# AbnerVictor/OOD-GAN-inversion

Hardware: AMD Instinct MI355X
Metric: 1024² face inversions/sec (100 W+ steps) (higher is better)
Workload: dtype f16-split (hi+lo f16 operands, f32 accumulate): 3 MFMA/product in every forward conv (fp32-equivalent), 2 in the input-gradient convs (back-propagated gradient rounded to f16 before each contraction, weights keep hi+lo); dL/dW+ vs the float64 reference 1.4e-5..3.6e-5 ('f16s': 1.3e-5..2.6e-5, the ref

## Files before the change

ood-gan-inversion_amd/csrc/common.hpp:

```cpp
#pragma once
#include <hip/hip_runtime.h>
#include <cstdio>
#include <cstdarg>
#include <functional>
#include <utility>
#include "../../include/oodgan.h"

namespace oodgan {
struct PlanRec;
extern thread_local PlanRec* tl_plan_rec;
extern int g_null_launch;
void plan_append(std::function<void()>&& f);
template <class F>
inline void launch_rec(F&& f) {
    f();
    if (__builtin_expect(tl_plan_rec != nullptr, 0)) plan_append(std::function<void()>(std::forward<F>(f)));
}
}
#undef hipLaunchKernelGGL
#define hipLaunchKernelGGL(kernelName, numBlocks, numThreads, memPerBlock, streamId, ...)                                        \
    ::oodgan::launch_rec([=]() {                                                                                                 \
        if (!::oodgan::g_null_launch) (kernelName)<<<(numBlocks), (numThreads), (memPerBlock), (streamId)>>>(__VA_ARGS__);      \
    })

namespace oodgan {

void set_error(const char* fmt, ...);

enum { OODGAN_TUN_S1_BIG_MIN_ITEMS = 0, OODGAN_TUN_S2_BIG_MIN_ITEMS, OODGAN_TUN_T2_BIG_MIN_ITEMS, OODGAN_TUN_BLURT_STRIP, OODGAN_TUN_BLUR_STRIP, OODGAN_TUN_UPVB_WAVES, OODGAN_TUN_FEWOUT_QUAD, OODGAN_TUN_TINY_MID_MAX, OODGAN_TUN_STRIPX_WAVES, OODGAN_TUN_COUNT };
long tunable(int id);

enum { OODGAN_DC_STRIPX = 0, OODGAN_DC_STRIP, OODGAN_DC_S1BIG, OODGAN_DC_S1V2, OODGAN_DC_S1PP, OODGAN_DC_TINY, OODGAN_DC_T2BIG,
       OODGAN_DC_T2V2, OODGAN_DC_T2GEN, OODGAN_DC_S2BIG, OODGAN_DC_S2V2, OODGAN_DC_S2GEN, OODGAN_DC_UPVB,
       OODGAN_DC_S1BIG_YS, OODGAN_DC_S2BIG_FUSE, OODGAN_DC_S2BIG_DOTXS,
       OODGAN_DC_S1BIG_G2, OODGAN_DC_S2BIG_G2, OODGAN_DC_STRIPX_G2, OODGAN_DC_S2BIG_XH, OODGAN_DC_S1BIG_XH,
       OODGAN_DC_COMPOSITE_MSE,
       OODGAN_DC_SSIM,
       OODGAN_DC_ROBUST,
       OODGAN_DC_AREA_POOL,
       OODGAN_DC_POOLED_PIXEL, OODGAN_DC_COUNT };
void count_dispatch(int id);

bool bound_device_ok(const char* what);

inline int check_launch(const char* what) {
    hipError_t e = hipGetLastError();
    if (e != hipSuccess) {
        set_error("%s: %s", what, hipGetErrorString(e));
        return OODGAN_E_LAUNCH;
    }
    return OODGAN_OK;
}

#define OODGAN_REQUIRE(cond, ...)          \
    do {                                    \
        if (!(cond)) {                      \
            oodgan::set_error(__VA_ARGS__); \
            return OODGAN_E_ARG;            \
        }                                   \
    } while (0)

constexpr float kSqrt2 = 1.4142135623730951f;
constexpr float kInvPos = 1.f / kSqrt2, kInvNeg = 1.f / (0.2f * kSqrt2);
constexpr int kWave = 64;

inline hipStream_t as_stream(void* s) { return reinterpret_cast<hipStream_t>(s); }

inline int stream_grid(long work_items, int block) {
    long g = (work_items + block - 1) / block;
    if (g > 2048) g = 2048;
    if (g < 1) g = 1;
    return static_cast<int>(g);
}

__device__ __forceinline__ float wave_sum(float v) {
#pragma unroll
    for (int o = 32; o > 0; o >>= 1) v += __shfl_xor(v, o, 64);
    return v;
}

__device__ __forceinline__ float row_sum16(const float* __restrict__ p, int n, int l) {
    float v[4];
// ... 119 lines not shown
```

ood-gan-inversion_amd/csrc/conv_f16s_s2big.hip:

```cpp
#include "conv_common.hpp"
#include "sform.hpp"
#include <cstdint>
#include <cstdlib>
#include <type_traits>

using namespace oodgan;

typedef _Float16 half8 __attribute__((ext_vector_type(8)));
typedef __attribute__((address_space(3))) void lds_void;

#ifdef OODGAN_CLOCK_STAMP
__device__ unsigned long long* g_s2big_stamp = nullptr;
__device__ long g_s2big_stamp_n = 0;
#define S2_STAMP(i) do { if (FUSE && (wave == 0 || wave == 7)) stv[i] = __builtin_amdgcn_s_memtime(); } while (0)
#else
#define S2_STAMP(i)
#endif

namespace {

constexpr int SB_ROWS = 9, SB_C = 33;
constexpr int SB_ROWSLOTS = 2 * SB_C * 4;
constexpr int SB_XSLOTS = SB_ROWS * SB_ROWSLOTS;
constexpr int SB_XPIECES = 40;
constexpr int SB_XBYTES = SB_XPIECES * 1024;

struct SPDims2 { int KC, Hq, Wq; long plane; };

__host__ __device__ inline SPDims2 sp_dims2(int C, int H, int W) {
    SPDims2 d;
    d.KC = (C + 15) / 16;
    d.Hq = (H + 7) / 8 * 8 + 2;
    d.Wq = (W + 31) / 32 * 32 + 2;
    d.plane = (long)d.Hq * d.Wq * 4;
    return d;
}

struct S2Big {
    oodgan_conv_args a;
    const uint4* xs;
    SPDims2 sp;
    const float* w_unscale;
    int Hout, Wout, tiles_x, tiles_y, mblocks, Mp;
    long out_plane;
    int ablate;
    oodgan_actbwd_fuse f;
    SDims yd;
};

template <int MH>
struct S2Cfg {
    static constexpr int RW = MH == 2 ? 2 : 1;
    static constexpr int NRG = 8 / RW;
    static constexpr int MBW = 64 * MH;
    static constexpr int TAPB = 4 * MBW * 16;
    static constexpr int PPT = TAPB / 1024;
    static constexpr int WA = 6 * PPT / 8, WB = (3 * PPT + 7) / 8;
    static constexpr int NA = 5 + WA, NB = 5 + WB;
    static constexpr int OFF_XA = 0, OFF_WA = SB_XBYTES, OFF_XB = OFF_WA + 6 * TAPB, OFF_WB = OFF_XB + SB_XBYTES;
    static constexpr int SMEM = OFF_WB + 3 * TAPB;
    static constexpr int OFF_CST = SMEM;
    static constexpr int SMEM_FUSE = SMEM + 8 * MBW * 4;
};

constexpr int vmcnt_imm(int n) { return ((n >> 4) & 3) << 14 | 0x0F70 | (n & 15); }

typedef _Float16 half2v __attribute__((ext_vector_type(2)));

template <bool DOT, int MH, bool FUSE = false, bool G2 = false>
__global__ __launch_bounds__(512) void conv_f16s_s2big_kernel(const S2Big p, const uint4* __restrict__ wpk16) {
    using C = S2Cfg<MH>;
    constexpr int RW = C::RW;
    extern __shared__ __attribute__((aligned(16))) unsigned char smem[];
    const oodgan_conv_args& a = p.a;
    const int tid = threadIdx.x, lane = tid & 63;
    const int wave = __builtin_amdgcn_readfirstlane(tid >> 6);
    const int l31 = lane & 31, half = lane >> 5;
    const int rg = wave % C::NRG, mh = wave / C::NRG;

#ifdef OODGAN_CLOCK_STAMP
    unsigned long long stv[8] = {0, 0, 0, 0, 0, 0, 0, 0};
#endif
    S2_STAMP(0);
    int w = xcd_remap(blockIdx.x, gridDim.x);
    const int mblk = w % p.mblocks;
    w /= p.mblocks;
    const int ntile = p.tiles_x * p.tiles_y;
    const int tile = w % ntile, b = w / ntile;
    const int ty = tile / p.tiles_x, tx = tile % p.tiles_x;
    const int r0 = ty * 8, c0 = tx * 32, m0 = mblk * C::MBW;
    const int H = p.Hout, W = p.Wout, M = a.M;

    const bool xh = G2 && a.x_hi_only == 2;
    unsigned offx[5];
    bool xok[5];
#pragma unroll
    for (int i = 0; i < 5; ++i) {
        int P = (wave + 8 * i) * 64 + lane;
        if (P >= SB_XSLOTS) P = SB_XSLOTS - 1;
        const int row = P / SB_ROWSLOTS, rem = P % SB_ROWSLOTS;
        const int px = rem / (SB_C * 4), q = rem % (SB_C * 4);
        const int c = q >> 2, s = ((q & 3) - ((c >> 2) & 3)) & 3;
        if (xh) {
            offx[i] = (unsigned)(((long)px * p.sp.plane + ((long)(r0 + row) * p.sp.Wq + (c0 + c)) * 2 + (s & 1)) * 16);
            xok[i] = s < 2;
        } else {
            offx[i] = (unsigned)(((long)px * p.sp.plane + ((long)(r0 + row) * p.sp.Wq + (c0 + c)) * 4 + s) * 16);
            xok[i] = true;
        }
    }
    const long plane_bytes = p.sp.plane * 16;
    const int grp = a.groups > 1 ? m0 / (M / a.groups) : 0;
    const unsigned char* xb = reinterpret_cast<const unsigned char*>(p.xs) + ((long)b * p.sp.KC + (long)grp * ((a.K + 15) / 16)) * 4 * plane_bytes;
    const unsigned char* wb = reinterpret_cast<const unsigned char*>(wpk16) + (long)m0 * 16;
    const unsigned lane16 = lane * 16;
    const long wchunk_bytes = (long)36 * p.Mp * 16;
    const long wrow_bytes = (long)p.Mp * 16;
    const int nchunk = (a.K + 15) / 16;
    const int nstage = 2 * nchunk;

    auto dma_piece = [&](int st, int j) {
        const int t = st >> 1, py = st & 1;
        if (j < 5) {
            unsigned char* dx_ = smem + (py ? C::OFF_XB : C::OFF_XA);
            const unsigned char* xsrc = xb + ((long)t * 4 + py * 2) * plane_bytes;
            if (!G2 || xok[j])
                __builtin_amdgcn_global_load_lds((const __attribute__((address_space(1))) void*)(xsrc + offx[j]),
                                                 (lds_void*)(dx_ + (wave + 8 * j) * 1024), 16, 0, 0);
            return;
        }
        const int i = j - 5;
        const int nw = py ? C::WB : C::WA, npieces = (py ? 3 : 6) * C::PPT;
        if (i >= nw) return;
        unsigned char* dw_ = smem + (py ? C::OFF_WB : C::OFF_WA);
        const unsigned char* wsrc = wb + (long)t * wchunk_bytes;
        int pw = wave + 8 * i;
        if (pw >= npieces) pw -= 8;
        const int sl = pw / C::PPT, q = pw % C::PPT;
        const int tap = py ? 3 + sl : (sl / 3) * 6 + sl % 3;
        const int row = (q * 64) / C::MBW, j0 = (q * 64) % C::MBW;
        const unsigned char* sb = wsrc + (long)(tap * 4 + row) * wrow_bytes + j0 * 16;
        __builtin_amdgcn_global_load_lds((const __attribute__((address_space(1))) void*)(sb + lane16), (lds_void*)(dw_ + pw * 1024), 16, 0, 0);
    };
    auto dma_stage = [&](int st) {
#pragma unroll
        for (int j = 0; j < C::NA; ++j) dma_piece(st, j);
    };

    f32x16 acc[2][RW];
#pragma unroll
    for (int mt = 0; mt < 2; ++mt)
#pragma unroll
        for (int nt = 0; nt < RW; ++nt)
#pragma unroll
            for (int r = 0; r < 16; ++r) acc[mt][nt][r] = 0.f;

    unsigned lrd[2][2];
#pragma unroll
    for (int dxs = 0; dxs < 2; ++dxs)
#pragma unroll
        for (int lo = 0; lo < 2; ++lo) {
            const int c = dxs + l31;
            lrd[dxs][lo] = c * 64 + (((half + 2 * lo + ((c >> 2) & 3)) & 3) << 4);
        }
    const unsigned lwf = (half * C::MBW + mh * 64 + l31) * 16;

    struct Frag { half8 ah[2], al[2], bh[RW], bl[RW]; };
    auto load_tap = [&](Frag& f, const unsigned char* lx, const unsigned char* lw, auto sl_c) {
        constexpr int sl = decltype(sl_c)::value;
        constexpr int arow = sl / 3, kx = sl % 3;
#pragma unroll
        for (int mt = 0; mt < 2; ++mt) {
            f.ah[mt] = *reinterpret_cast<const half8*>(lw + sl * C::TAPB + (0 * 2) * C::MBW * 16 + mt * 32 * 16);
            f.al[mt] = *reinterpret_cast<const half8*>(lw + sl * C::TAPB + (1 * 2) * C::MBW * 16 + mt * 32 * 16);
        }
#pragma unroll
        for (int nt = 0; nt < RW; ++nt) {
            const unsigned char* xr = lx + ((rg * RW + nt + arow) * 2 + (kx & 1)) * (SB_C * 64);
            f.bh[nt] = *reinterpret_cast<const half8*>(xr + lrd[kx >> 1][0]);
            if (!G2) f.bl[nt] = *reinterpret_cast<const half8*>(xr + lrd[kx >> 1][1]);
        }
    };
    auto mfma_tap = [&](const Frag& f) {
#pragma unroll
        for (int mt = 0; mt < 2; ++mt)
#pragma unroll
            for (int nt = 0; nt < RW; ++nt) acc[mt][nt] = __builtin_amdgcn_mfma_f32_32x32x16_f16(f.ah[mt], f.bh[nt], acc[mt][nt], 0, 0, 0);
        if (!G2) {
#pragma unroll
        for (int mt = 0; mt < 2; ++mt)
#pragma unroll
            for (int nt = 0; nt < RW; ++nt) acc[mt][nt] = __builtin_amdgcn_mfma_f32_32x32x16_f16(f.ah[mt], f.bl[nt], acc[mt][nt], 0, 0, 0);
        }
#pragma unroll
        for (int mt = 0; mt < 2; ++mt)
#pragma unroll
            for (int nt = 0; nt < RW; ++nt) acc[mt][nt] = __builtin_amdgcn_mfma_f32_32x32x16_f16(f.al[mt], f.bh[nt], acc[mt][nt], 0, 0, 0);
    };
#define S2B_IC(n) std::integral_constant<int, n>{}
#define S2B_SB() __builtin_amdgcn_sched_barrier(0)

    constexpr bool EARLY = FUSE && MH == 1;
    float eq0 = 0.f, eq1 = 0.f, eq2 = 0.f, enz = 0.f, edv[EARLY ? 2 : 1][16];
    bool eok = false;
    if constexpr (EARLY) {
        static_assert(!EARLY || RW == 1, "one row per wave");
        const oodgan_actbwd_fuse& f = p.f;
        const int px = c0 + l31, py_ = r0 + rg;
        const long HW = (long)H * W, pix = (long)py_ * W + px;
        eok = py_ < H && px < W;
        if (eok) {
            if (f.g_rgb) {
                const float* gr = f.g_rgb + (long)b * 3 * HW + pix;
                eq0 = gr[0]; eq1 = gr[HW]; eq2 = gr[2 * HW];
            }
            if (f.noise) enz = (f.noise_w ? f.noise_w[0] : 1.f) * f.noise[(long)(f.noise_batch > 1 ? b : 0) * HW + pix];
        }
        if (a.dotx_sform) {
#pragma unroll
            for (int mt = 0; mt < 2; ++mt)
#pragma unroll
                for (int blk = 0; blk < 2; ++blk) {
                    const int kc = min((m0 + mh * 64 + mt * 32) / 16 + blk, p.yd.KC - 1);
                    const unsigned char* rec = reinterpret_cast<const unsigned char*>(a.dotx) +
                        sform_unit(p.yd, b, kc, min(py_, H - 1), min(px, W - 1), 0) * 16 + 8 * half;
#pragma unroll
                    for (int sl = 0; sl < 4; ++sl) {
                        const float2 t = *reinterpret_cast<const float2*>(rec + 16 * sl);
                        edv[EARLY ? mt : 0][8 * blk + 2 * sl] = t.x;
                        edv[EARLY ? mt : 0][8 * blk + 2 * sl + 1] = t.y;
                    }
                }
        } else {
#pragma unroll
            for (int mt = 0; mt < 2; ++mt) {
                const float* dr = a.dotx + ((long)b * M + m0 + mh * 64 + mt * 32) * HW + pix;
#pragma unroll
                for (int r = 0; r < 16; ++r) {
                    const int ch = (r & 3) + 8 * (r >> 2) + 4 * half;
                    edv[EARLY ? mt : 0][r] = (eok && m0 + mh * 64 + mt * 32 + ch < M) ? dr[(long)ch * HW] : 0.f;
                }
            }
        }
    }

    float cv[8] = {0.f, 0.f, 0.f, 0.f, 0.f, 0.f, 0.f, 1.f};
    if constexpr (FUSE) {
        const oodgan_actbwd_fuse& f = p.f;
        if (tid < C::MBW) {
            const int m = min(m0 + tid, M - 1);
            cv[0] = a.out_scale ? a.out_scale[(long)b * a.out_scale_stride + m] : 1.f;
            if (f.g_rgb) {
                cv[1] = f.w_rgb[0 * M + m];
                cv[2] = f.w_rgb[1 * M + m];
                cv[3] = f.w_rgb[2 * M + m];
                cv[4] = f.s_rgb[(long)b * f.s_rgb_stride + m];
            }
            if (f.bias) cv[5] = f.bias[m];
            cv[6] = f.dscale[(long)b * f.dscale_stride + m];
            if (a.dotx_sform) {
                const float sc = a.dotx_scale[(long)b * a.dotx_scale_stride + m];
                cv[7] = sc != 0.f ? 1.f / sc : 0.f;
            }
        }
    }
    dma_stage(0);
    if constexpr (FUSE) {
        if (tid < C::MBW) {
            const oodgan_actbwd_fuse& f = p.f;
            float* cst = reinterpret_cast<float*>(smem + C::OFF_CST);
            const bool mok = m0 + tid < M;
            cst[0 * C::MBW + tid] = mok ? cv[0] : 0.f;
            cst[1 * C::MBW + tid] = mok ? cv[1] * f.rgb_scale : 0.f;
            cst[2 * C::MBW + tid] = mok ? cv[2] * f.rgb_scale : 0.f;
            cst[3 * C::MBW + tid] = mok ? cv[3] * f.rgb_scale : 0.f;
            cst[4 * C::MBW + tid] = mok ? cv[4] : 0.f;
            cst[5 * C::MBW + tid] = mok ? cv[5] : 0.f;
            cst[6 * C::MBW + tid] = mok ? cv[6] * f.mul2[1] : 0.f;
            cst[7 * C::MBW + tid] = mok ? cv[7] : 0.f;
            __builtin_amdgcn_s_waitcnt(0xC07F);
        }
    }
    S2_STAMP(1);
    for (int st = 0; st < nstage; ++st) {
        const int py = st & 1;
        __builtin_amdgcn_s_waitcnt(vmcnt_imm(0));
        __builtin_amdgcn_s_barrier();
        const bool pf = st + 1 < nstage && !(p.ablate & 2);
        if (p.ablate & 1) { if (pf) dma_stage(st + 1); continue; }
        const unsigned char* lx = smem + (py ? C::OFF_XB : C::OFF_XA);
        const unsigned char* lw = smem + (py ? C::OFF_WB : C::OFF_WA) + lwf;
        Frag f0, f1;
        if (MH == 2 && pf) dma_stage(st + 1);
#define S2B_DMA(j) if (MH == 1 && pf) dma_piece(st + 1, (j));
        load_tap(f0, lx, lw, S2B_IC(0));
        S2B_SB();
        if (py == 0) {
            load_tap(f1, lx, lw, S2B_IC(1)); S2B_DMA(0) S2B_DMA(1) S2B_SB(); mfma_tap(f0); S2B_SB();
            load_tap(f0, lx, lw, S2B_IC(2)); S2B_DMA(2) S2B_DMA(3) S2B_SB(); mfma_tap(f1); S2B_SB();
            load_tap(f1, lx, lw, S2B_IC(3)); S2B_DMA(4) S2B_SB(); mfma_tap(f0); S2B_SB();
            load_tap(f0, lx, lw, S2B_IC(4)); S2B_DMA(5) S2B_SB(); mfma_tap(f1); S2B_SB();
            load_tap(f1, lx, lw, S2B_IC(5)); S2B_DMA(6) S2B_SB(); mfma_tap(f0); S2B_SB();
            S2B_DMA(7) S2B_SB();
            mfma_tap(f1);
        } else {
            load_tap(f1, lx, lw, S2B_IC(1)); S2B_DMA(0) S2B_DMA(1) S2B_DMA(2) S2B_DMA(3) S2B_SB(); mfma_tap(f0); S2B_SB();
            load_tap(f0, lx, lw, S2B_IC(2)); S2B_DMA(4) S2B_DMA(5) S2B_DMA(6) S2B_DMA(7) S2B_SB(); mfma_tap(f1); S2B_SB();
            S2B_DMA(8) S2B_DMA(9) S2B_DMA(10) S2B_SB();
            mfma_tap(f0);
        }
#undef S2B_DMA
    }
    __builtin_amdgcn_s_barrier();
    S2_STAMP(2);
#undef S2B_IC
#undef S2B_SB

    if constexpr (FUSE) {
        static_assert(DOT, "the fused epilogue includes the dot");
        const oodgan_actbwd_fuse& f = p.f;
        float* red = reinterpret_cast<float*>(smem);
        float* cst = reinterpret_cast<float*>(smem + C::OFF_CST);
        const float us = (p.w_unscale ? p.w_unscale[0] : 1.f) * (a.in_mul2 ? a.in_mul2[0] : 1.f);
        const float rscale = f.mul2[1];
        const int px = c0 + l31;
        const long HW = (long)H * W;
        const float nw = f.noise ? (f.noise_w ? f.noise_w[0] : 1.f) : 0.f;
        float q0[RW], q1[RW], q2[RW], nzv[RW];
        bool okr[RW];
#pragma unroll
        for (int nt = 0; nt < RW; ++nt) {
            const int py_ = r0 + rg * RW + nt;
            okr[nt] = py_ < H && px < W;
            q0[nt] = q1[nt] = q2[nt] = nzv[nt] = 0.f;
            if constexpr (EARLY) {
                okr[nt] = eok; q0[nt] = eq0; q1[nt] = eq1; q2[nt] = eq2; nzv[nt] = enz;
            } else if (okr[nt]) {
                const long pix = (long)py_ * W + px;
                if (f.g_rgb) {
                    const float* gr = f.g_rgb + (long)b * 3 * HW + pix;
                    q0[nt] = gr[0]; q1[nt] = gr[HW]; q2[nt] = gr[2 * HW];
                }
                if (f.noise) nzv[nt] = nw * f.noise[(long)(f.noise_batch > 1 ? b : 0) * HW + pix];
            }
        }
        float vmaxv = 0.f;
#pragma unroll
        for (int mt = 0; mt < 2; ++mt) {
            if (MH == 2) __builtin_amdgcn_sched_barrier(0);
            const int chb = mh * 64 + mt * 32;
            float dv[RW][16];
            if (a.dotx_sform) {
#pragma unroll
                for (int nt = 0; nt < RW; ++nt) {
                    float raw[16];
                    if constexpr (EARLY) {
#pragma unroll
                        for (int i = 0; i < 16; ++i) raw[i] = edv[EARLY ? mt : 0][i];
                    } else {
                        const int py_ = r0 + rg * RW + nt;
#pragma unroll
                        for (int blk = 0; blk < 2; ++blk) {
                            const int kc = min((m0 + chb) / 16 + blk, p.yd.KC - 1);
                            const unsigned char* rec = reinterpret_cast<const unsigned char*>(a.dotx) +
                                sform_unit(p.yd, b, kc, min(py_, H - 1), min(px, W - 1), 0) * 16 + 8 * half;
#pragma unroll
                            for (int sl = 0; sl < 4; ++sl) {
                                const float2 t = *reinterpret_cast<const float2*>(rec + 16 * sl);
                                raw[8 * blk + 2 * sl] = t.x;
                                raw[8 * blk + 2 * sl + 1] = t.y;
                            }
                        }
                    }
#pragma unroll
                    for (int r = 0; r < 16; ++r) {
// ... 278 lines not shown

namespace oodgan {

int launch_s2_big(const oodgan_conv_args& a_in, const void* wpk16, const float* unscale, hipStream_t st) {
    S2Big p;
    p.a = a_in;
    oodgan_conv_args& a = p.a;
    p.Hout = (a.Hin - 1) / 2;
    p.Wout = (a.Win - 1) / 2;
    if (a.out_pitch == 0) a.out_pitch = p.Wout;
    p.out_plane = (long)p.Hout * a.out_pitch;
    p.xs = reinterpret_cast<const uint4*>(a.x);
    p.sp = sp_dims2(a.K * (a.groups > 1 ? a.groups : 1), p.Hout, p.Wout);
    p.w_unscale = unscale;
    p.tiles_y = (p.Hout + 7) / 8;
    p.tiles_x = (p.Wout + 31) / 32;
    p.Mp = (a.M + 63) / 64 * 64;
    const long items128 = (long)p.tiles_x * p.tiles_y * a.B * (a.M / 128);
    const bool mh2 = (a.M % 128) == 0 && items128 >= 256;
    p.mblocks = mh2 ? a.M / 128 : (a.M + 63) / 64;
    if (a.dotx) {
        OODGAN_REQUIRE(a.dot_part != nullptr, "conv3x3: dotx without dot_part");
        OODGAN_REQUIRE(a.dot_nparts == p.tiles_x * p.tiles_y, "conv3x3 f16s S2: dot_nparts %d != %d", a.dot_nparts, p.tiles_x * p.tiles_y);
    }
    OODGAN_REQUIRE((long)a.M * p.out_plane * 4 < (1L << 32), "conv3x3 S2 big: plane too large");
    const bool fuse = a.fuse != nullptr;
    p.yd = sform_dims(a.M, p.Hout, p.Wout);
    if (fuse) {
        p.f = *a.fuse;
        OODGAN_REQUIRE(a.dotx && a.dot_part && p.f.ys && p.f.part_r && p.f.part_max && p.f.dscale && p.f.mul2 && (a.M % 32) == 0,
                       "conv3x3 S2 fused activation backward: needs dotx, ys, part_r, part_max, dscale, mul2 and M %% 32 == 0");
        OODGAN_REQUIRE(!p.f.g_rgb || (p.f.w_rgb && p.f.s_rgb && p.f.part_t), "conv3x3 S2 fused: rgb branch needs w_rgb, s_rgb and part_t");
        OODGAN_REQUIRE(p.f.noise == nullptr || p.f.noise_batch == 1 || p.f.noise_batch == a.B, "conv3x3 S2 fused: noise_batch");
        OODGAN_REQUIRE(p.f.nmax >= (long)a.B * p.tiles_x * p.tiles_y * p.mblocks * 8, "conv3x3 S2 fused: part_max too small");
    }
    OODGAN_REQUIRE(p.sp.plane * 32 < (1L << 32), "conv3x3 S2 big: input plane too large");
#ifdef OODGAN_DEBUG_ABLATE
    static const int abl = getenv("OODGAN_S2BIG_ABLATE") ? atoi(getenv("OODGAN_S2BIG_ABLATE")) : 0;
    p.ablate = abl;
#else
    p.ablate = 0;
#endif
    const long total = (long)p.tiles_x * p.tiles_y * a.B * p.mblocks;
    OODGAN_REQUIRE(total > 0 && total < (1L << 31), "conv3x3: grid too large");
    static bool once = ((void)hipFuncSetAttribute(reinterpret_cast<const void*>(&conv_f16s_s2big_kernel<true, 2>), hipFuncAttributeMaxDynamicSharedMemorySize, S2Cfg<2>::SMEM),
                        (void)hipFuncSetAttribute(reinterpret_cast<const void*>(&conv_f16s_s2big_kernel<false, 2>), hipFuncAttributeMaxDynamicSharedMemorySize, S2Cfg<2>::SMEM),
                        (void)hipFuncSetAttribute(reinterpret_cast<const void*>(&conv_f16s_s2big_kernel<true, 1>), hipFuncAttributeMaxDynamicSharedMemorySize, S2Cfg<1>::SMEM),
                        (void)hipFuncSetAttribute(reinterpret_cast<const void*>(&conv_f16s_s2big_kernel<false, 1>), hipFuncAttributeMaxDynamicSharedMemorySize, S2Cfg<1>::SMEM),
                        (void)hipFuncSetAttribute(reinterpret_cast<const void*>(&conv_f16s_s2big_kernel<true, 2, true>), hipFuncAttributeMaxDynamicSharedMemorySize, S2Cfg<2>::SMEM_FUSE),
                        (void)hipFuncSetAttribute(reinterpret_cast<const void*>(&conv_f16s_s2big_kernel<true, 1, true>), hipFuncAttributeMaxDynamicSharedMemorySize, S2Cfg<1>::SMEM_FUSE),
                        (void)hipFuncSetAttribute(reinterpret_cast<const void*>(&conv_f16s_s2big_kernel<true, 2, false, true>), hipFuncAttributeMaxDynamicSharedMemorySize, S2Cfg<2>::SMEM),
                        (void)hipFuncSetAttribute(reinterpret_cast<const void*>(&conv_f16s_s2big_kernel<true, 1, false, true>), hipFuncAttributeMaxDynamicSharedMemorySize, S2Cfg<1>::SMEM),
                        (void)hipFuncSetAttribute(reinterpret_cast<const void*>(&conv_f16s_s2big_kernel<true, 2, true, true>), hipFuncAttributeMaxDynamicSharedMemorySize, S2Cfg<2>::SMEM_FUSE),
                        (void)hipFuncSetAttribute(reinterpret_cast<const void*>(&conv_f16s_s2big_kernel<true, 1, true, true>), hipFuncAttributeMaxDynamicSharedMemorySize, S2Cfg<1>::SMEM_FUSE), true);
    (void)once;
    const uint4* w16 = reinterpret_cast<const uint4*>(wpk16);
    const bool g2 = a.x_hi_only != 0 && a.dotx != nullptr;
    OODGAN_REQUIRE(a.x_hi_only != 2 || (g2 && a.groups <= 1), "conv3x3 S2 big: hi-only input records (x_hi_only = 2) need dotx (the two-instruction instances) and no groups");
    if (g2) {
        count_dispatch(OODGAN_DC_S2BIG_G2);
        if (a.x_hi_only == 2) count_dispatch(OODGAN_DC_S2BIG_XH);
        if (fuse) {
            if (mh2) hipLaunchKernelGGL((conv_f16s_s2big_kernel<true, 2, true, true>), dim3((unsigned)total), dim3(512), S2Cfg<2>::SMEM_FUSE, st, p, w16);
            else hipLaunchKernelGGL((conv_f16s_s2big_kernel<true, 1, true, true>), dim3((unsigned)total), dim3(512), S2Cfg<1>::SMEM_FUSE, st, p, w16);
        } else if (mh2) hipLaunchKernelGGL((conv_f16s_s2big_kernel<true, 2, false, true>), dim3((unsigned)total), dim3(512), S2Cfg<2>::SMEM, st, p, w16);
        else hipLaunchKernelGGL((conv_f16s_s2big_kernel<true, 1, false, true>), dim3((unsigned)total), dim3(512), S2Cfg<1>::SMEM, st, p, w16);
    } else if (fuse) {
        if (mh2) hipLaunchKernelGGL((conv_f16s_s2big_kernel<true, 2, true>), dim3((unsigned)total), dim3(512), S2Cfg<2>::SMEM_FUSE, st, p, w16);
        else hipLaunchKernelGGL((conv_f16s_s2big_kernel<true, 1, true>), dim3((unsigned)total), dim3(512), S2Cfg<1>::SMEM_FUSE, st, p, w16);
    } else if (mh2) {
        if (a.dotx) hipLaunchKernelGGL((conv_f16s_s2big_kernel<true, 2>), dim3((unsigned)total), dim3(512), S2Cfg<2>::SMEM, st, p, w16);
        else hipLaunchKernelGGL((conv_f16s_s2big_kernel<false, 2>), dim3((unsigned)total), dim3(512), S2Cfg<2>::SMEM, st, p, w16);
    } else {
        if (a.dotx) hipLaunchKernelGGL((conv_f16s_s2big_kernel<true, 1>), dim3((unsigned)total), dim3(512), S2Cfg<1>::SMEM, st, p, w16);
        else hipLaunchKernelGGL((conv_f16s_s2big_kernel<false, 1>), dim3((unsigned)total), dim3(512), S2Cfg<1>::SMEM, st, p, w16);
    }
    return check_launch("conv3x3_f16s_s2big");
}

}
```

ood-gan-inversion_amd/csrc/runtime.hip:

```cpp
#include "common.hpp"
#include <atomic>
#include <cstdlib>
#include <cstring>
#include <new>

namespace oodgan {
static thread_local char g_err[512] = "";
void set_error(const char* fmt, ...) {
    va_list ap;
    va_start(ap, fmt);
    vsnprintf(g_err, sizeof(g_err), fmt, ap);
    va_end(ap);
}
}

namespace oodgan {
namespace {
struct Tunable { const char* name; const char* env; long def; std::atomic<long> val; std::atomic<int> init; };
Tunable g_tun[OODGAN_TUN_COUNT] = {
    {"s1_big_min_items", "OODGAN_S1_BIG_MIN_ITEMS", 128, {0}, {0}},
    {"s2_big_min_items", "OODGAN_S2_BIG_MIN_ITEMS", 128, {0}, {0}},
    {"t2_big_min_items", "OODGAN_T2_BIG_MIN_ITEMS", 128, {0}, {0}},
    {"blurt_strip", "OODGAN_BLURT_STRIP", 1, {0}, {0}},
    {"blur_strip", "OODGAN_BLUR_STRIP", 1, {0}, {0}},
    {"upvb_waves", "OODGAN_UPVB_WAVES", 12, {0}, {0}},
    {"fewout_quad", "OODGAN_FEWOUT_QUAD", 1, {0}, {0}},
    {"tiny_mid_max", "OODGAN_TINY_MID_MAX", 1024, {0}, {0}},
    {"stripx_waves", "OODGAN_STRIPX_WAVES", 4, {0}, {0}},
};
}
long tunable(int id) {
    Tunable& t = g_tun[id];
    if (!t.init.load(std::memory_order_acquire)) {
        const char* e = getenv(t.env);
        t.val.store(e ? atol(e) : t.def, std::memory_order_relaxed);
        t.init.store(1, std::memory_order_release);
    }
    return t.val.load(std::memory_order_relaxed);
}
}

extern "C" int oodgan_set_tunable(const char* name, long value) {
    OODGAN_REQUIRE(name != nullptr, "set_tunable: null name");
    for (int i = 0; i < oodgan::OODGAN_TUN_COUNT; ++i)
        if (strcmp(name, oodgan::g_tun[i].name) == 0) {
            oodgan::g_tun[i].val.store(value, std::memory_order_relaxed);
            oodgan::g_tun[i].init.store(1, std::memory_order_release);
            return OODGAN_OK;
        }
    oodgan::set_error("set_tunable: unknown tunable '%s'", name);
    return OODGAN_E_ARG;
}
extern "C" long oodgan_get_tunable(const char* name) {
    if (name)
        for (int i = 0; i < oodgan::OODGAN_TUN_COUNT; ++i)
            if (strcmp(name, oodgan::g_tun[i].name) == 0) return oodgan::tunable(i);
    return -1;
}

namespace oodgan {
bool bound_device_ok(const char* what) {
    static std::atomic<int> bound{-1};
    int dev = 0;
    if (hipGetDevice(&dev) != hipSuccess) {
        (void)hipGetLastError();
        set_error("%s: no current HIP device", what);
        return false;
    }
    int expected = -1;
    if (bound.compare_exchange_strong(expected, dev, std::memory_order_acq_rel) || expected == dev) return true;
    set_error("%s: liboodgan_hip.so is bound to HIP device %d (its first use in this process) but device %d is current — one process per GPU "
              "(select the device with HIP_VISIBLE_DEVICES or torch.cuda.set_device before the first call)", what, expected, dev);
    return false;
}
}

namespace oodgan {
namespace {
const char* const g_dc_name[OODGAN_DC_COUNT] = {"stripx", "strip", "s1big", "s1v2", "s1pp", "tiny", "t2big", "t2v2", "t2gen", "s2big", "s2v2", "s2gen", "upvb", "s1big_ys", "s2big_fuse", "s2big_dotx_sform", "s1big_g2", "s2big_g2", "stripx_g2", "s2big_xh", "s1big_xh", "composite_mse", "ssim", "robust", "area_pool", "pooled_pixel"};
std::atomic<long> g_dc[OODGAN_DC_COUNT];
}
// ... 98 lines not shown
```

ood-gan-inversion_amd/csrc/upfirdn2d.hip:

```cpp
#include "common.hpp"

using namespace oodgan;

namespace {

struct UfdArgs {
    const float* x;
    const float* k;
    float* y;
    const float* bias;
    const float* noise;
    const float* noise_w;
    int planes, C;
    int in_h, in_w, in_pitch;
    int out_h, out_w, out_pitch;
    int kh, kw, up_x, up_y, down_x, down_y, pad_x0, pad_y0;
    int noise_batch, act;
};

__global__ __launch_bounds__(256) void generic_kernel(const UfdArgs a) {
    const long total = (long)a.planes * a.out_h * a.out_w;
    const long in_plane = (long)a.in_h * a.in_pitch, out_plane = (long)a.out_h * a.out_pitch;
    for (long e = blockIdx.x * (long)blockDim.x + threadIdx.x; e < total; e += (long)gridDim.x * blockDim.x) {
        const int ox = (int)(e % a.out_w);
        const int oy = (int)((e / a.out_w) % a.out_h);
        const long pl = e / ((long)a.out_w * a.out_h);
        const float* xp = a.x + pl * in_plane;
        float acc = 0.f;
        for (int ky = 0; ky < a.kh; ++ky) {
            const int u = oy * a.down_y + ky - a.pad_y0;
            if (u < 0 || u % a.up_y) continue;
            const int iy = u / a.up_y;
            if (iy >= a.in_h) continue;
            for (int kx = 0; kx < a.kw; ++kx) {
                const int v = ox * a.down_x + kx - a.pad_x0;
                if (v < 0 || v % a.up_x) continue;
                const int ix = v / a.up_x;
                if (ix >= a.in_w) continue;
                acc += a.k[(a.kh - 1 - ky) * a.kw + (a.kw - 1 - kx)] * xp[(long)iy * a.in_pitch + ix];
            }
        }
        if (a.noise) {
            const long b = pl / a.C;
            acc += (a.noise_w ? a.noise_w[0] : 1.f) * a.noise[(a.noise_batch > 1 ? b : 0) * (long)a.out_h * a.out_w + (long)oy * a.out_w + ox];
        }
        if (a.bias) acc += a.bias[pl % a.C];
        if (a.act == OODGAN_ACT_LRELU) acc = (acc > 0.f ? acc : 0.2f * acc) * kSqrt2;
        a.y[pl * out_plane + (long)oy * a.out_pitch + ox] = acc;
    }
}

__global__ __launch_bounds__(256) void down2_k4_kernel(const UfdArgs a) {
    __shared__ float kf[16];
    if (threadIdx.x < 16) kf[threadIdx.x] = a.k[15 - threadIdx.x];
    __syncthreads();
    const long total = (long)a.planes * a.out_h * a.out_w;
    const long in_plane = (long)a.in_h * a.in_pitch, out_plane = (long)a.out_h * a.out_pitch;
    for (long e = blockIdx.x * 256L + threadIdx.x; e < total; e += (long)gridDim.x * 256) {
        const int ox = (int)(e % a.out_w);
        const int oy = (int)((e / a.out_w) % a.out_h);
        const long pl = e / ((long)a.out_w * a.out_h);
        const float* xp = a.x + pl * in_plane;
        const int y0 = 2 * oy - a.pad_y0, x0 = 2 * ox - a.pad_x0;
        float v[16];
#pragma unroll
        for (int ky = 0; ky < 4; ++ky)
#pragma unroll
            for (int kx = 0; kx < 4; ++kx)
                v[ky * 4 + kx] = xp[(long)min(max(y0 + ky, 0), a.in_h - 1) * a.in_pitch + min(max(x0 + kx, 0), a.in_w - 1)];
        float acc = 0.f;
#pragma unroll
        for (int ky = 0; ky < 4; ++ky)
#pragma unroll
            for (int kx = 0; kx < 4; ++kx) {
                const int iy = y0 + ky, ix = x0 + kx;
                if (iy >= 0 && iy < a.in_h && ix >= 0 && ix < a.in_w) acc += kf[ky * 4 + kx] * v[ky * 4 + kx];
            }
        a.y[pl * out_plane + (long)oy * a.out_pitch + ox] = acc;
    }
}

constexpr int FT_H = 32, FT_W = 64, FK = 4;
constexpr int FL_H = FT_H + FK - 1, FL_W = FT_W + FK - 1;
constexpr int FL_P = FL_W + 1;

__global__ __launch_bounds__(256) void fir_tile_kernel(const UfdArgs a, int tiles_x, int tiles_y) {
    __shared__ float t[FL_H * FL_P];
    __shared__ float kf[FK * FK];
    int w = blockIdx.x;
    const int tx_ = w % tiles_x; w /= tiles_x;
    const int ty_ = w % tiles_y; w /= tiles_y;
    const long pl = w;
    const int oy0 = ty_ * FT_H, ox0 = tx_ * FT_W;
    const long in_plane = (long)a.in_h * a.in_pitch, out_plane = (long)a.out_h * a.out_pitch;
    const float* xp = a.x + pl * in_plane;
    if (threadIdx.x < FK * FK) {
        const int ky = threadIdx.x / FK, kx = threadIdx.x % FK;
        kf[threadIdx.x] = (ky < a.kh && kx < a.kw) ? a.k[(a.kh - 1 - ky) * a.kw + (a.kw - 1 - kx)] : 0.f;
    }
    const int iy0 = oy0 - a.pad_y0, ix0 = ox0 - a.pad_x0;
    {
        constexpr int NF = (FL_H * FL_W + 255) / 256;
        float fv[NF];
#pragma unroll
        for (int i = 0; i < NF; ++i) {
            const int e = min((int)threadIdx.x + 256 * i, FL_H * FL_W - 1);
            const int iy = iy0 + e / FL_W, ix = ix0 + e % FL_W;
            fv[i] = xp[(long)min(max(iy, 0), a.in_h - 1) * a.in_pitch + min(max(ix, 0), a.in_w - 1)];
        }
#pragma unroll
        for (int i = 0; i < NF; ++i) {
            const int e = (int)threadIdx.x + 256 * i;
            if (e >= FL_H * FL_W) continue;
            const int r = e / FL_W, c = e % FL_W;
            const int iy = iy0 + r, ix = ix0 + c;
            t[r * FL_P + c] = (iy >= 0 && iy < a.in_h && ix >= 0 && ix < a.in_w) ? fv[i] : 0.f;
        }
    }
    __syncthreads();
    const int tx = threadIdx.x & 15, ty = threadIdx.x >> 4;
    float kr[FK * FK];
#pragma unroll
    for (int i = 0; i < FK * FK; ++i) kr[i] = kf[i];
    const long b = pl / a.C;
    const float bv = a.bias ? a.bias[pl % a.C] : 0.f;
    const float nw = a.noise ? (a.noise_w ? a.noise_w[0] : 1.f) : 0.f;
    const float* np = a.noise ? a.noise + (a.noise_batch > 1 ? b : 0) * (long)a.out_h * a.out_w : nullptr;
    float nzv[2][4];
#pragma unroll
    for (int rr = 0; rr < 2; ++rr)
#pragma unroll
        for (int j = 0; j < 4; ++j) {
            const int oy = min(oy0 + ty + rr * 16, a.out_h - 1), ox = min(ox0 + 4 * tx + j, a.out_w - 1);
            nzv[rr][j] = *(np ? np + (long)oy * a.out_w + ox : xp);
        }
#pragma unroll
    for (int rr = 0; rr < 2; ++rr) {
        const int r = ty + rr * 16;
        float o[4] = {0.f, 0.f, 0.f, 0.f};
#pragma unroll
        for (int ky = 0; ky < FK; ++ky) {
            float row[4 + FK - 1];
#pragma unroll
            for (int j = 0; j < 4 + FK - 1; ++j) row[j] = t[(r + ky) * FL_P + 4 * tx + j];
#pragma unroll
            for (int kx = 0; kx < FK; ++kx)
#pragma unroll
                for (int j = 0; j < 4; ++j) o[j] += kr[ky * FK + kx] * row[j + kx];
        }
        const int oy = oy0 + r;
        if (oy >= a.out_h) continue;
#pragma unroll
        for (int j = 0; j < 4; ++j) {
            const int ox = ox0 + 4 * tx + j;
            if (ox >= a.out_w) continue;
            float v = o[j];
            if (np) v += nw * nzv[rr][j];
            v += bv;
            if (a.act == OODGAN_ACT_LRELU) v = (v > 0.f ? v : 0.2f * v) * kSqrt2;
            a.y[pl * out_plane + (long)oy * a.out_pitch + ox] = v;
        }
    }
}

int run(UfdArgs& a, int pad_x1, int pad_y1, hipStream_t st) {
    OODGAN_REQUIRE(a.x && a.k && a.y, "upfirdn2d: null tensor");
    OODGAN_REQUIRE(a.planes > 0 && a.in_h > 0 && a.in_w > 0 && a.kh > 0 && a.kw > 0, "upfirdn2d: bad shape");
    OODGAN_REQUIRE(a.up_x >= 1 && a.up_y >= 1 && a.down_x >= 1 && a.down_y >= 1, "upfirdn2d: up/down must be >= 1");
    a.out_h = (a.in_h * a.up_y + a.pad_y0 + pad_y1 - a.kh) / a.down_y + 1;
    a.out_w = (a.in_w * a.up_x + a.pad_x0 + pad_x1 - a.kw) / a.down_x + 1;
    OODGAN_REQUIRE(a.out_h > 0 && a.out_w > 0, "upfirdn2d: empty output (%d x %d)", a.out_h, a.out_w);
    if (a.in_pitch == 0) a.in_pitch = a.in_w;
    if (a.out_pitch == 0) a.out_pitch = a.out_w;
    OODGAN_REQUIRE(a.in_pitch >= a.in_w && a.out_pitch >= a.out_w, "upfirdn2d: pitch smaller than width");
    const bool tiled = a.up_x == 1 && a.up_y == 1 && a.down_x == 1 && a.down_y == 1 && a.kh <= FK && a.kw <= FK &&
                       (long)a.out_h * a.out_w >= 64 * 64;
    if (tiled) {
        const int tiles_x = (a.out_w + FT_W - 1) / FT_W, tiles_y = (a.out_h + FT_H - 1) / FT_H;
        const long nb = (long)tiles_x * tiles_y * a.planes;
        OODGAN_REQUIRE(nb < (1L << 31), "upfirdn2d: grid too large");
        hipLaunchKernelGGL(fir_tile_kernel, dim3((unsigned)nb), dim3(256), 0, st, a, tiles_x, tiles_y);
    } else if (a.up_x == 1 && a.up_y == 1 && a.down_x == 2 && a.down_y == 2 && a.kh == 4 && a.kw == 4 && !a.noise && !a.bias &&
               a.act == OODGAN_ACT_NONE) {
        const long total = (long)a.planes * a.out_h * a.out_w;
        hipLaunchKernelGGL(down2_k4_kernel, dim3(stream_grid(total, 256)), dim3(256), 0, st, a);
    } else {
        const long total = (long)a.planes * a.out_h * a.out_w;
        hipLaunchKernelGGL(generic_kernel, dim3(stream_grid(total, 256)), dim3(256), 0, st, a);
    }
    return check_launch("upfirdn2d");
}

}

extern "C" int oodgan_upfirdn2d(const float* x, const float* kernel, float* y, int planes, int in_h, int in_w, int in_pitch,
                                int out_pitch, int kh, int kw, int up_x, int up_y, int down_x, int down_y, int pad_x0,
                                int pad_x1, int pad_y0, int pad_y1, void* stream) {
    UfdArgs a{};
    a.x = x; a.k = kernel; a.y = y;
    a.planes = planes; a.C = 1;
    a.in_h = in_h; a.in_w = in_w; a.in_pitch = in_pitch; a.out_pitch = out_pitch;
    a.kh = kh; a.kw = kw; a.up_x = up_x; a.up_y = up_y; a.down_x = down_x; a.down_y = down_y;
    a.pad_x0 = pad_x0; a.pad_y0 = pad_y0;
    a.act = OODGAN_ACT_NONE; a.noise_batch = 1;
    return run(a, pad_x1, pad_y1, as_stream(stream));
}

extern "C" int oodgan_blur_bias_act(const float* x, const float* kernel, float* y, int B, int C, int in_h, int in_w,
                                    int in_pitch, int kh, int kw, int pad0, int pad1, const float* bias, const float* noise,
                                    int noise_batch, const float* noise_w, int act, void* stream) {
    OODGAN_REQUIRE(B > 0 && C > 0, "blur_bias_act: bad batch/channels");
    OODGAN_REQUIRE(noise == nullptr || noise_batch == 1 || noise_batch == B, "blur_bias_act: noise_batch");
    UfdArgs a{};
    a.x = x; a.k = kernel; a.y = y;
    a.planes = B * C; a.C = C;
    a.in_h = in_h; a.in_w = in_w; a.in_pitch = in_pitch; a.out_pitch = 0;
    a.kh = kh; a.kw = kw; a.up_x = a.up_y = a.down_x = a.down_y = 1;
    a.pad_x0 = pad0; a.pad_y0 = pad0;
    a.bias = bias; a.noise = noise; a.noise_w = noise_w; a.noise_batch = noise_batch; a.act = act;
    return run(a, pad1, pad1, as_stream(stream));
}
```

Before: 7.897.

## Add resident-operand stride-2 conv path and vectorized down2 FIR kernel

Adds a resident-operand variant of the fused MH=1 stride-2 conv kernel. It DMAs every stage's input and weight tiles into LDS up front and then runs the MFMA stages behind staged vmcnt waits, replacing the per-stage load/wait loop. This is meant to overlap all global loads with compute for small-K layers, at the cost of a larger LDS footprint and so possibly lower occupancy. Separately, it adds a vectorized downsample-by-2 4x4 FIR kernel that computes four outputs per thread from float4 row loads, cutting redundant scalar loads. Both paths are gated by new tunables that default on.

Result: no change. 7.957 (median of 5 runs) (+0.8%).

```diff
diff --git a/ood-gan-inversion_amd/csrc/common.hpp b/ood-gan-inversion_amd/csrc/common.hpp
--- a/ood-gan-inversion_amd/csrc/common.hpp
+++ b/ood-gan-inversion_amd/csrc/common.hpp
@@ -27,7 +27,7 @@
 
 void set_error(const char* fmt, ...);
 
-enum { OODGAN_TUN_S1_BIG_MIN_ITEMS = 0, OODGAN_TUN_S2_BIG_MIN_ITEMS, OODGAN_TUN_T2_BIG_MIN_ITEMS, OODGAN_TUN_BLURT_STRIP, OODGAN_TUN_BLUR_STRIP, OODGAN_TUN_UPVB_WAVES, OODGAN_TUN_FEWOUT_QUAD, OODGAN_TUN_TINY_MID_MAX, OODGAN_TUN_STRIPX_WAVES, OODGAN_TUN_COUNT };
+enum { OODGAN_TUN_S1_BIG_MIN_ITEMS = 0, OODGAN_TUN_S2_BIG_MIN_ITEMS, OODGAN_TUN_T2_BIG_MIN_ITEMS, OODGAN_TUN_BLURT_STRIP, OODGAN_TUN_BLUR_STRIP, OODGAN_TUN_UPVB_WAVES, OODGAN_TUN_FEWOUT_QUAD, OODGAN_TUN_TINY_MID_MAX, OODGAN_TUN_STRIPX_WAVES, OODGAN_TUN_DOWN2_VEC, OODGAN_TUN_S2_RESIDENT, OODGAN_TUN_COUNT };
 long tunable(int id);
 
 enum { OODGAN_DC_STRIPX = 0, OODGAN_DC_STRIP, OODGAN_DC_S1BIG, OODGAN_DC_S1V2, OODGAN_DC_S1PP, OODGAN_DC_TINY, OODGAN_DC_T2BIG,
diff --git a/ood-gan-inversion_amd/csrc/conv_f16s_s2big.hip b/ood-gan-inversion_amd/csrc/conv_f16s_s2big.hip
--- a/ood-gan-inversion_amd/csrc/conv_f16s_s2big.hip
+++ b/ood-gan-inversion_amd/csrc/conv_f16s_s2big.hip
@@ -63,14 +63,25 @@
     static constexpr int SMEM_FUSE = SMEM + 8 * MBW * 4;
 };
 
+constexpr int RS_XSLOTS = SB_ROWS * 2 * SB_C * 2;
+constexpr int RS_XPIECES = 19;
+constexpr int RS_XREG = RS_XPIECES * 1024;
+constexpr int RS_TAPB = 4096;
+constexpr int RS_OFF_W = 4 * RS_XREG;
+constexpr int RS_OFF_CST = RS_OFF_W + 18 * RS_TAPB;
+constexpr int RS_SMEM = RS_OFF_CST + 8 * 64 * 4;
+constexpr int RS_NA = 6, RS_NB = 5;
+
 constexpr int vmcnt_imm(int n) { return ((n >> 4) & 3) << 14 | 0x0F70 | (n & 15); }
 
 typedef _Float16 half2v __attribute__((ext_vector_type(2)));
 
-template <bool DOT, int MH, bool FUSE = false, bool G2 = false>
+template <bool DOT, int MH, bool FUSE = false, bool G2 = false, bool RES = false>
 __global__ __launch_bounds__(512) void conv_f16s_s2big_kernel(const S2Big p, const uint4* __restrict__ wpk16) {
     using C = S2Cfg<MH>;
     constexpr int RW = C::RW;
+    static_assert(!RES || (MH == 1 && FUSE && G2), "the resident-operand form exists for the fused two-instruction MH = 1 instance");
+    constexpr int OFF_CST = RES ? RS_OFF_CST : C::OFF_CST;
     extern __shared__ __attribute__((aligned(16))) unsigned char smem[];
     const oodgan_conv_args& a = p.a;
     const int tid = threadIdx.x, lane = tid & 63;
@@ -94,6 +105,18 @@
     const bool xh = G2 && a.x_hi_only == 2;
     unsigned offx[5];
     bool xok[5];
+    if constexpr (RES) {
+#pragma unroll
+        for (int i = 0; i < 3; ++i) {
+            int P = min(wave + 8 * i, RS_XPIECES - 1) * 64 + lane;
+            if (P >= RS_XSLOTS) P = RS_XSLOTS - 1;
+            const int run = P / (2 * SB_C), q = P % (2 * SB_C);
+            const int row = run >> 1, px = run & 1, c = q >> 1, u = (q ^ (c >> 3)) & 1;
+            offx[i] = (unsigned)(((long)px * p.sp.plane + ((long)(r0 + row) * p.sp.Wq + (c0 + c)) * 2 + u) * 16);
+            xok[i] = true;
+        }
+        offx[3] = offx[4] = 0; xok[3] = xok[4] = false;
+    } else {
 #pragma unroll
     for (int i = 0; i < 5; ++i) {
         int P = (wave + 8 * i) * 64 + lane;
@@ -108,6 +131,7 @@
             offx[i] = (unsigned)(((long)px * p.sp.plane + ((long)(r0 + row) * p.sp.Wq + (c0 + c)) * 4 + s) * 16);
             xok[i] = true;
         }
+    }
     }
     const long plane_bytes = p.sp.plane * 16;
     const int grp = a.groups > 1 ? m0 / (M / a.groups) : 0;
@@ -181,6 +205,38 @@
             if (!G2) f.bl[nt] = *reinterpret_cast<const half8*>(xr + lrd[kx >> 1][1]);
         }
     };
+    const unsigned lrr0 = l31 * 32 + ((half ^ (l31 >> 3)) & 1) * 16, lrr1 = (l31 + 1) * 32 + ((half ^ ((l31 + 1) >> 3)) & 1) * 16;
+    auto load_tap_r = [&](Frag& f, const unsigned char* lx, const unsigned char* lw, auto py_c, auto sl_c) {
+        constexpr int sl = decltype(sl_c)::value, py = decltype(py_c)::value;
+        constexpr int arow = sl / 3, kx = sl % 3, tap = py ? 3 + sl : (sl / 3) * 6 + sl % 3;
+#pragma unroll
+        for (int mt = 0; mt < 2; ++mt) {
+            f.ah[mt] = *reinterpret_cast<const half8*>(lw + tap * RS_TAPB + (0 * 2) * 64 * 16 + mt * 32 * 16);
+            f.al[mt] = *reinterpret_cast<const half8*>(lw + tap * RS_TAPB + (1 * 2) * 64 * 16 + mt * 32 * 16);
+        }
+        f.bh[0] = *reinterpret_cast<const half8*>(lx + ((rg + arow) * 2 + (kx & 1)) * (SB_C * 32) + ((kx >> 1) ? lrr1 : lrr0));
+    };
+    auto dma_stage_r = [&](int st) {
+        const int t = st >> 1, py = st & 1;
+        const unsigned char* xsrc = xb + ((long)t * 4 + py * 2) * plane_bytes;
+#pragma unroll
+        for (int i = 0; i < 3; ++i)
+            __builtin_amdgcn_global_load_lds((const __attribute__((address_space(1))) void*)(xsrc + offx[i]),
+                                             (lds_void*)(smem + st * RS_XREG + min(wave + 8 * i, RS_XPIECES - 1) * 1024), 16, 0, 0);
+        const unsigned char* wsrc = wb + (long)t * wchunk_bytes;
+        const int nw = py ? 2 : 3;
+#pragma unroll
+        for (int i = 0; i < 3; ++i) {
+            if (i >= nw) break;
+            int pw = wave + 8 * i;
+            if (pw >= (py ? 12 : 24)) pw -= 8;
+            const int sl = pw >> 2, row = pw & 3;
+            const int tap = py ? 3 + sl : (sl / 3) * 6 + sl % 3;
+            const unsigned char* sb = wsrc + (long)(tap * 4 + row) * wrow_bytes;
+            __builtin_amdgcn_global_load_lds((const __attribute__((address_space(1))) void*)(sb + lane16),
+                                             (lds_void*)(smem + RS_OFF_W + (t * 9 + tap) * RS_TAPB + row * 1024), 16, 0, 0);
+        }
+    };
     auto mfma_tap = [&](const Frag& f) {
 #pragma unroll
         for (int mt = 0; mt < 2; ++mt)
@@ -264,11 +320,17 @@
             }
         }
     }
-    dma_stage(0);
-    if constexpr (FUSE) {
+    if constexpr (RES) {
+        S2B_SB();
+        for (int st = 0; st < nstage; ++st) dma_stage_r(st);
+        S2B_SB();
+    } else {
+        dma_stage(0);
+    }
+    auto park_cst = [&]() {
         if (tid < C::MBW) {
             const oodgan_actbwd_fuse& f = p.f;
-            float* cst = reinterpret_cast<float*>(smem + C::OFF_CST);
+            float* cst = reinterpret_cast<float*>(smem + OFF_CST);
             const bool mok = m0 + tid < M;
             cst[0 * C::MBW + tid] = mok ? cv[0] : 0.f;
             cst[1 * C::MBW + tid] = mok ? cv[1] * f.rgb_scale : 0.f;
@@ -280,8 +342,45 @@
             cst[7 * C::MBW + tid] = mok ? cv[7] : 0.f;
             __builtin_amdgcn_s_waitcnt(0xC07F);
         }
-    }
+    };
+    if constexpr (FUSE && !RES) park_cst();
     S2_STAMP(1);
+    if constexpr (RES) {
+        auto stage_a = [&](int t) {
+            const unsigned char* lx = smem + (2 * t) * RS_XREG;
+            const unsigned char* lw = smem + RS_OFF_W + t * 9 * RS_TAPB + lwf;
+            Frag f0, f1;
+            load_tap_r(f0, lx, lw, S2B_IC(0), S2B_IC(0));
+            S2B_SB();
+            load_tap_r(f1, lx, lw, S2B_IC(0), S2B_IC(1)); S2B_SB(); mfma_tap(f0); S2B_SB();
+            load_tap_r(f0, lx, lw, S2B_IC(0), S2B_IC(2)); S2B_SB(); mfma_tap(f1); S2B_SB();
+            load_tap_r(f1, lx, lw, S2B_IC(0), S2B_IC(3)); S2B_SB(); mfma_tap(f0); S2B_SB();
+            load_tap_r(f0, lx, lw, S2B_IC(0), S2B_IC(4)); S2B_SB(); mfma_tap(f1); S2B_SB();
+            load_tap_r(f1, lx, lw, S2B_IC(0), S2B_IC(5)); S2B_SB(); mfma_tap(f0); S2B_SB();
+            mfma_tap(f1);
+        };
+        auto stage_b = [&](int t) {
+            const unsigned char* lx = smem + (2 * t + 1) * RS_XREG;
+            const unsigned char* lw = smem + RS_OFF_W + t * 9 * RS_TAPB + lwf;
+            Frag f0, f1;
+            load_tap_r(f0, lx, lw, S2B_IC(1), S2B_IC(0));
+            S2B_SB();
+            load_tap_r(f1, lx, lw, S2B_IC(1), S2B_IC(1)); S2B_SB(); mfma_tap(f0); S2B_SB();
+            load_tap_r(f0, lx, lw, S2B_IC(1), S2B_IC(2)); S2B_SB(); mfma_tap(f1); S2B_SB();
+            mfma_tap(f0);
+        };
+#define S2B_WAIT(n) do { S2B_SB(); __builtin_amdgcn_s_waitcnt(vmcnt_imm(n)); __builtin_amdgcn_s_barrier(); S2B_SB(); } while (0)
+        if (nchunk == 2) {
+            S2B_WAIT(RS_NB + RS_NA + RS_NB); stage_a(0);
+            S2B_WAIT(RS_NA + RS_NB); stage_b(0);
+            S2B_WAIT(RS_NB); stage_a(1);
+            S2B_WAIT(0); stage_b(1);
+        } else {
+            S2B_WAIT(RS_NB); stage_a(0);
+            S2B_WAIT(0); stage_b(0);
+        }
+#undef S2B_WAIT
+    } else
     for (int st = 0; st < nstage; ++st) {
         const int py = st & 1;
         __builtin_amdgcn_s_waitcnt(vmcnt_imm(0));
@@ -311,6 +410,7 @@
         }
 #undef S2B_DMA
     }
+    if constexpr (RES) park_cst();
     __builtin_amdgcn_s_barrier();
     S2_STAMP(2);
 #undef S2B_IC
@@ -320,7 +420,7 @@
         static_assert(DOT, "the fused epilogue includes the dot");
         const oodgan_actbwd_fuse& f = p.f;
         float* red = reinterpret_cast<float*>(smem);
-        float* cst = reinterpret_cast<float*>(smem + C::OFF_CST);
+        float* cst = reinterpret_cast<float*>(smem + OFF_CST);
         const float us = (p.w_unscale ? p.w_unscale[0] : 1.f) * (a.in_mul2 ? a.in_mul2[0] : 1.f);
         const float rscale = f.mul2[1];
         const int px = c0 + l31;
@@ -705,7 +805,8 @@
                         (void)hipFuncSetAttribute(reinterpret_cast<const void*>(&conv_f16s_s2big_kernel<true, 2, false, true>), hipFuncAttributeMaxDynamicSharedMemorySize, S2Cfg<2>::SMEM),
                         (void)hipFuncSetAttribute(reinterpret_cast<const void*>(&conv_f16s_s2big_kernel<true, 1, false, true>), hipFuncAttributeMaxDynamicSharedMemorySize, S2Cfg<1>::SMEM),
                         (void)hipFuncSetAttribute(reinterpret_cast<const void*>(&conv_f16s_s2big_kernel<true, 2, true, true>), hipFuncAttributeMaxDynamicSharedMemorySize, S2Cfg<2>::SMEM_FUSE),
-                        (void)hipFuncSetAttribute(reinterpret_cast<const void*>(&conv_f16s_s2big_kernel<true, 1, true, true>), hipFuncAttributeMaxDynamicSharedMemorySize, S2Cfg<1>::SMEM_FUSE), true);
+                        (void)hipFuncSetAttribute(reinterpret_cast<const void*>(&conv_f16s_s2big_kernel<true, 1, true, true>), hipFuncAttributeMaxDynamicSharedMemorySize, S2Cfg<1>::SMEM_FUSE),
+                        (void)hipFuncSetAttribute(reinterpret_cast<const void*>(&conv_f16s_s2big_kernel<true, 1, true, true, true>), hipFuncAttributeMaxDynamicSharedMemorySize, RS_SMEM), true);
     (void)once;
     const uint4* w16 = reinterpret_cast<const uint4*>(wpk16);
     const bool g2 = a.x_hi_only != 0 && a.dotx != nullptr;
@@ -714,7 +815,9 @@
         count_dispatch(OODGAN_DC_S2BIG_G2);
         if (a.x_hi_only == 2) count_dispatch(OODGAN_DC_S2BIG_XH);
         if (fuse) {
+            const bool res = !mh2 && a.x_hi_only == 2 && a.K <= 32 && a.groups <= 1 && tunable(OODGAN_TUN_S2_RESIDENT) != 0;
             if (mh2) hipLaunchKernelGGL((conv_f16s_s2big_kernel<true, 2, true, true>), dim3((unsigned)total), dim3(512), S2Cfg<2>::SMEM_FUSE, st, p, w16);
+            else if (res) hipLaunchKernelGGL((conv_f16s_s2big_kernel<true, 1, true, true, true>), dim3((unsigned)total), dim3(512), RS_SMEM, st, p, w16);
             else hipLaunchKernelGGL((conv_f16s_s2big_kernel<true, 1, true, true>), dim3((unsigned)total), dim3(512), S2Cfg<1>::SMEM_FUSE, st, p, w16);
         } else if (mh2) hipLaunchKernelGGL((conv_f16s_s2big_kernel<true, 2, false, true>), dim3((unsigned)total), dim3(512), S2Cfg<2>::SMEM, st, p, w16);
         else hipLaunchKernelGGL((conv_f16s_s2big_kernel<true, 1, false, true>), dim3((unsigned)total), dim3(512), S2Cfg<1>::SMEM, st, p, w16);
diff --git a/ood-gan-inversion_amd/csrc/runtime.hip b/ood-gan-inversion_amd/csrc/runtime.hip
--- a/ood-gan-inversion_amd/csrc/runtime.hip
+++ b/ood-gan-inversion_amd/csrc/runtime.hip
@@ -27,6 +27,8 @@
     {"fewout_quad", "OODGAN_FEWOUT_QUAD", 1, {0}, {0}},
     {"tiny_mid_max", "OODGAN_TINY_MID_MAX", 1024, {0}, {0}},
     {"stripx_waves", "OODGAN_STRIPX_WAVES", 4, {0}, {0}},
+    {"down2_vec", "OODGAN_DOWN2_VEC", 1, {0}, {0}},
+    {"s2_resident", "OODGAN_S2_RESIDENT", 1, {0}, {0}},
 };
 }
 long tunable(int id) {
diff --git a/ood-gan-inversion_amd/csrc/upfirdn2d.hip b/ood-gan-inversion_amd/csrc/upfirdn2d.hip
--- a/ood-gan-inversion_amd/csrc/upfirdn2d.hip
+++ b/ood-gan-inversion_amd/csrc/upfirdn2d.hip
@@ -1,4 +1,5 @@
 #include "common.hpp"
+#include <cstdint>
 
 using namespace oodgan;
 
@@ -77,6 +78,49 @@
                 if (iy >= 0 && iy < a.in_h && ix >= 0 && ix < a.in_w) acc += kf[ky * 4 + kx] * v[ky * 4 + kx];
             }
         a.y[pl * out_plane + (long)oy * a.out_pitch + ox] = acc;
+    }
+}
+
+__global__ __launch_bounds__(256) void down2_k4_vec_kernel(const UfdArgs a) {
+    __shared__ float kf[16];
+    if (threadIdx.x < 16) kf[threadIdx.x] = a.k[15 - threadIdx.x];
+    __syncthreads();
+    const int qw = a.out_w >> 2;
+    const long total = (long)a.planes * a.out_h * qw;
+    const long in_plane = (long)a.in_h * a.in_pitch, out_plane = (long)a.out_h * a.out_pitch;
+    for (long e = blockIdx.x * 256L + threadIdx.x; e < total; e += (long)gridDim.x * 256) {
+        const int q = (int)(e % qw);
+        const int oy = (int)((e / qw) % a.out_h);
+        const long pl = e / ((long)qw * a.out_h);
+        const float* xp = a.x + pl * in_plane;
+        const int y0 = 2 * oy - 1, xl = 8 * q - 1, xr = 8 * q + 8;
+        const bool lok = xl >= 0, rok = xr < a.in_w;
+        float r[4][10];
+        bool yok[4];
+#pragma unroll
+        for (int ky = 0; ky < 4; ++ky) {
+            yok[ky] = y0 + ky >= 0 && y0 + ky < a.in_h;
+            const float* rp = xp + (long)min(max(y0 + ky, 0), a.in_h - 1) * a.in_pitch;
+            const float4 m0 = *reinterpret_cast<const float4*>(rp + 8 * q), m1 = *reinterpret_cast<const float4*>(rp + 8 * q + 4);
+            r[ky][0] = rp[max(xl, 0)];
+            r[ky][1] = m0.x; r[ky][2] = m0.y; r[ky][3] = m0.z; r[ky][4] = m0.w;
+            r[ky][5] = m1.x; r[ky][6] = m1.y; r[ky][7] = m1.z; r[ky][8] = m1.w;
+            r[ky][9] = rp[min(xr, a.in_w - 1)];
+        }
+        float o[4];
+#pragma unroll
+        for (int j = 0; j < 4; ++j) {
+            float acc = 0.f;
+#pragma unroll
+            for (int ky = 0; ky < 4; ++ky)
+#pragma unroll
+                for (int kx = 0; kx < 4; ++kx) {
+                    const int c = 2 * j + kx;
+                    if (yok[ky] && (c != 0 || lok) && (c != 9 || rok)) acc += kf[ky * 4 + kx] * r[ky][c];
+                }
+            o[j] = acc;
+        }
+        *reinterpret_cast<float4*>(a.y + pl * out_plane + (long)oy * a.out_pitch + 4 * q) = make_float4(o[0], o[1], o[2], o[3]);
     }
 }
 
@@ -183,7 +227,11 @@
     } else if (a.up_x == 1 && a.up_y == 1 && a.down_x == 2 && a.down_y == 2 && a.kh == 4 && a.kw == 4 && !a.noise && !a.bias &&
                a.act == OODGAN_ACT_NONE) {
         const long total = (long)a.planes * a.out_h * a.out_w;
-        hipLaunchKernelGGL(down2_k4_kernel, dim3(stream_grid(total, 256)), dim3(256), 0, st, a);
+        const bool vec = a.in_w % 8 == 0 && a.pad_x0 == 1 && a.pad_y0 == 1 && 2 * a.out_w == a.in_w && a.in_pitch % 4 == 0 &&
+                         a.out_pitch % 4 == 0 && ((uintptr_t)a.x & 15) == 0 && ((uintptr_t)a.y & 15) == 0 &&
+                         tunable(OODGAN_TUN_DOWN2_VEC) != 0;
+        if (vec) hipLaunchKernelGGL(down2_k4_vec_kernel, dim3(stream_grid(total / 4, 256)), dim3(256), 0, st, a);
+        else hipLaunchKernelGGL(down2_k4_kernel, dim3(stream_grid(total, 256)), dim3(256), 0, st, a);
     } else {
         const long total = (long)a.planes * a.out_h * a.out_w;
         hipLaunchKernelGGL(generic_kernel, dim3(stream_grid(total, 256)), dim3(256), 0, st, a);
```
